# MasonFeurer/VoxelRayTracing

Hardware: AMD Instinct MI355X
Metric: Mrays/s at 1920x1080, 1 primary + 1 shadow ray (higher is better)
Workload: dtype f32

## Files before the change

### voxelraytracing_amd/csrc/vrt_kernels.hip

```cpp
#include <hip/hip_ext.h>

#include <atomic>

#include "vrt_tile.h"
#include "vrt_path_common.h"

namespace vrt {


template <int MARCH, bool LDS_ROOTS, bool STATS, bool SHADOW>
__global__ void __launch_bounds__(256) primary_tile_kernel(FrameParams P) {
    extern __shared__ uint32_t smem[];
    uint32_t *s_liquid = smem, *s_roots = smem + 24;
    unsigned long long *s_acc = reinterpret_cast<unsigned long long *>(smem + 8);
    uint32_t *s_hits = smem + 22;
    if (STATS && threadIdx.x < 6) s_acc[threadIdx.x] = 0ull;
    if (threadIdx.x == 0) *s_hits = 0u;
    stage_lds(P, s_roots, s_liquid, LDS_ROOTS);

    const uint32_t lane = threadIdx.x & 63u;
    uint32_t t_local = blockIdx.x * (blockDim.x >> 6) + (threadIdx.x >> 6);
    const bool live = t_local < P.tiles_local;
    if (!SHADOW && P.tile_order && live) t_local = P.tile_order[t_local];
    MarchResult R;
// ... 33 lines not shown
                    P.hits[blockIdx.x * 256u + base + rank] =
                        make_uint4(slot, __float_as_uint(so.x), __float_as_uint(so.y), __float_as_uint(so.z));
                }
            }
        }
        if (STATS && P.steps) P.steps[slot] = R.iters;
        if (!SHADOW && P.tile_cost) {
            uint32_t trips = R.trips;
#pragma unroll
            for (int o = 32; o > 0; o >>= 1) trips = max(trips, (uint32_t)__shfl_xor((int)trips, o, 64));
            if (lane == 0) P.tile_cost[t_local] = trips;
        }
    }
    if (STATS) {
        block_add(s_acc, 0, R.iters);
        block_add(s_acc, 1, R.visits);
        block_add(s_acc, 2, R.hit ? 1ull : 0ull);
    }
    if (SHADOW || STATS) {
        __syncthreads();
        if (threadIdx.x == 0) {
            if (SHADOW) P.blk_counts[blockIdx.x] = *s_hits;
            if (STATS) {
                atomicAdd(&P.counters[kCtrSteps], s_acc[0]);
                atomicAdd(&P.counters[kCtrVisits], s_acc[1]);
                atomicAdd(&P.counters[kCtrPrimarySteps], s_acc[0]);
                atomicAdd(&P.counters[kCtrPrimaryVisits], s_acc[1]);
                atomicAdd(&P.counters[kCtrHits], s_acc[2]);
            }
        }
    }
}

template <int MARCH, bool LDS_ROOTS, bool STATS>
__global__ void __launch_bounds__(256) shadow_kernel(FrameParams P) {
    extern __shared__ uint32_t smem[];
    uint32_t *s_liquid = smem, *s_roots = smem + 24;
    unsigned long long *s_acc = reinterpret_cast<unsigned long long *>(smem + 8);
    const uint32_t count = P.blk_counts[blockIdx.x];
    if (!STATS && count == 0u) return;
    if (STATS && threadIdx.x < 6) s_acc[threadIdx.x] = 0ull;
    stage_lds(P, s_roots, s_liquid, LDS_ROOTS);

    const bool active = threadIdx.x < count;
    if (!STATS && (threadIdx.x & ~63u) >= count) return;
    MarchResult R;
    R.iters = 0; R.visits = 0; R.hit = false;
    uint32_t slot = 0;
    if (active) {
        const uint4 rec = P.hits[blockIdx.x * 256u + threadIdx.x];
        slot = rec.x;
        const V3 so{__uint_as_float(rec.y), __uint_as_float(rec.z), __uint_as_float(rec.w)};
        const V3 sd = normalize_wave(V3{P.sun_local[0] - so.x, P.sun_local[1] - so.y, P.sun_local[2] - so.z});
        R = march<MARCH, LDS_ROOTS, STATS>(P, s_roots, s_liquid, so, sd);
        if (R.hit) {
            uint4 t = P.out[slot];
            t.x = __float_as_uint(__uint_as_float(t.x) * kShadowFactor);
            t.y = __float_as_uint(__uint_as_float(t.y) * kShadowFactor);
            t.z = __float_as_uint(__uint_as_float(t.z) * kShadowFactor);
            t.w |= VRT_ID_SHADOWED;
            P.out[slot] = t;
        }
        if (STATS && P.steps) P.steps[slot] |= R.iters << 16;
    }
    if (STATS) {
        block_add(s_acc, 0, active ? R.iters : 0u);
        block_add(s_acc, 1, active ? R.visits : 0u);
        __syncthreads();
        if (threadIdx.x == 0 && s_acc[0]) {
            atomicAdd(&P.counters[kCtrSteps], s_acc[0]);
            atomicAdd(&P.counters[kCtrVisits], s_acc[1]);
        }
    }
}


template <int MARCH, bool LDS_ROOTS, bool STATS, int WAVES, bool PROBE = false>
__global__ void __launch_bounds__(64 * WAVES) primary_shadow_wave_kernel(FrameParams P) {
    extern __shared__ uint32_t smem[];
    uint32_t *s_liquid = smem, *s_roots = smem + 24;
    unsigned long long *s_acc = reinterpret_cast<unsigned long long *>(smem + 8);
    if (STATS && threadIdx.x < 6) s_acc[threadIdx.x] = 0ull;
    unsigned long long t0 = 0, r0 = 0;
    if (PROBE) {
        t0 = __builtin_amdgcn_s_memtime();
        r0 = __builtin_amdgcn_s_memrealtime();
    }
    stage_lds(P, s_roots, s_liquid, LDS_ROOTS);

    const uint32_t lane = threadIdx.x & 63u;
    uint32_t t_local = blockIdx.x * (uint32_t)WAVES + (threadIdx.x >> 6);
    if (P.tile_order && t_local < P.tiles_local) t_local = P.tile_order[t_local];
    MarchResult R, S;
    R.iters = 0; R.visits = 0; R.hit = false;
    S.iters = 0; S.visits = 0; S.hit = false;
    R.trips = 0; S.trips = 0;
    if (t_local < P.tiles_local) {
        trace_tile<MARCH, LDS_ROOTS, STATS>(P, s_roots, s_liquid, t_local, lane, R, S);
        if (P.tile_cost) {
            uint32_t trips = R.trips + S.trips;
#pragma unroll
            for (int o = 32; o > 0; o >>= 1) trips = max(trips, (uint32_t)__shfl_xor((int)trips, o, 64));
            if (lane == 0) P.tile_cost[t_local] = trips;
        }
    }
    if (PROBE) {
        const unsigned long long t1 = __builtin_amdgcn_s_memtime(), r1 = __builtin_amdgcn_s_memrealtime();
// ... 546 lines not shown
```

### voxelraytracing_amd/csrc/vrt_march.h

```cpp
#pragma once

#include "vrt_device.h"


namespace vrt {

__device__ __forceinline__ int trunc2i(float x) {
    int r;
    asm("v_cvt_i32_f32 %0, %1" : "=v"(r) : "v"(x));
    return r;
}

constexpr uint32_t kBandLo = 0x30800000u;
constexpr uint32_t kBandSpan = 0x4E800000u - kBandLo;
__device__ __forceinline__ bool in_band(float x) { return (__float_as_uint(x) & 0x7FFFFFFFu) - kBandLo <= kBandSpan; }
__device__ __forceinline__ bool in_band3(V3 v) {
    const uint32_t a = (__float_as_uint(v.x) & 0x7FFFFFFFu) - kBandLo, b = (__float_as_uint(v.y) & 0x7FFFFFFFu) - kBandLo,
                   c = (__float_as_uint(v.z) & 0x7FFFFFFFu) - kBandLo;
    return max(max(a, b), c) <= kBandSpan;
}
__device__ __forceinline__ float rcp_refined(float d) {
    const float r = __builtin_amdgcn_rcpf(d);
    const float e = __builtin_fmaf(-d, r, 1.0f);
    return __builtin_fmaf(e, r, r);
// ... 341 lines not shown

__device__ __forceinline__ uint32_t mad_i24(int a, uint32_t uniform_b, uint32_t c) {
    uint32_t r;
    asm("v_mad_i32_i24 %0, %1, %2, %3" : "=v"(r) : "v"(a), "s"(uniform_b), "v"(c));
    return r;
}

__device__ __forceinline__ uint32_t bfi(uint32_t mask, uint32_t a, uint32_t b) {
    uint32_t r;
    asm("v_bitop3_b32 %0, %1, %2, %3 bitop3:0xca" : "=v"(r) : "v"(mask), "v"(a), "v"(b));
    return r;
}

template <uint32_t MASK>
__device__ __forceinline__ uint32_t low_bits_of(uint32_t a, uint32_t b) {
    static_assert(MASK <= 64u, "an inline constant");
    uint32_t r;
    asm("v_bitop3_b32 %0, %1, %2, %3 bitop3:0xca" : "=v"(r) : "n"(MASK), "v"(a), "v"(b));
    return r;
}
__device__ __forceinline__ uint32_t or_and(uint32_t a, uint32_t b, uint32_t c_mask_reg) {
    uint32_t r;
    asm("v_bitop3_b32 %0, %1, %2, %3 bitop3:0xf8" : "=v"(r) : "v"(a), "v"(b), "v"(c_mask_reg));
    return r;
}

__device__ __forceinline__ float abs_mul(float a, float b) {
    float r;
    asm("v_mul_f32_e64 %0, |%1|, %2" : "=v"(r) : "v"(a), "v"(b));
    return r;
}

__device__ __forceinline__ int flr2i(float x) {
    int r;
    asm("v_cvt_flr_i32_f32 %0, %1" : "=v"(r) : "v"(x));
    return r;
}
__device__ __forceinline__ float min3_f32(float a, float b, float c) {
    float r;
    asm("v_min3_f32 %0, %1, %2, %3" : "=v"(r) : "v"(a), "v"(b), "v"(c));
    return r;
}
__device__ __forceinline__ uint32_t min3_u32(uint32_t a, uint32_t b, uint32_t c) {
    uint32_t r;
    asm("v_min3_u32 %0, %1, %2, %3" : "=v"(r) : "v"(a), "v"(b), "v"(c));
    return r;
}

__device__ __forceinline__ bool finite3(V3 v) {
    return ((__float_as_uint(v.x) & 0x7F800000u) != 0x7F800000u) && ((__float_as_uint(v.y) & 0x7F800000u) != 0x7F800000u) &&
           ((__float_as_uint(v.z) & 0x7F800000u) != 0x7F800000u);
}

template <bool STATS, bool CAMERA = false>
__device__ __forceinline__ MarchResult march_grid(const FrameParams &P, const uint32_t *s_liquid, V3 origin, V3 dir) {
    MarchResult R;
    R.hit = false;
    R.pos = V3{0.f, 0.f, 0.f};
    R.norm = V3{0.f, 0.f, 0.f};
    R.water_dist = 0.0f;
    R.voxel = 0u;
    R.iters = 0u;
    R.visits = 0u;
    R.trips = 0u;

    const bool mx = dir.x >= 0.0f, my = dir.y >= 0.0f, mz = dir.z >= 0.0f;
    const bool careful = CAMERA ? ((P.cam_origin_facts & kCamNotFinite) != 0u || __ballot(!finite3(dir)) != 0ull)
                                : __ballot(!(finite3(origin) && finite3(dir))) != 0ull;

    V3 pos = origin;
    const bool nudge = CAMERA ? (P.cam_origin_facts & kCamOnPlane) != 0u
                              : (pos.x - floorf(pos.x) < 0.001f || pos.y - floorf(pos.y) < 0.001f || pos.z - floorf(pos.z) < 0.001f);
    if (nudge) {
        pos.x += 0.001f * dir.x;
        pos.y += 0.001f * dir.y;
        pos.z += 0.001f * dir.z;
    }
    const float world_max = P.world_max;
    if (CAMERA && !(P.cam_origin_facts & kCamOnPlane)) {
        if (P.cam_origin_facts & kCamOutside) return R;
    } else if ((pos.x <= 0.0f || pos.y <= 0.0f || pos.z <= 0.0f) || (pos.x >= world_max || pos.y >= world_max || pos.z >= world_max))
        return R;

    const V3 unit = unit_steps(dir);
    float ux = fabsf(unit.x), uy = fabsf(unit.y), uz = fabsf(unit.z);
    asm("" : "+v"(ux), "+v"(uy), "+v"(uz));
    constexpr uint32_t kTwo23 = 0x4B000000u;
    uint32_t mxm = kTwo23 | (mx ? 0x007FFFFFu : 0u), mym = kTwo23 | (my ? 0x007FFFFFu : 0u), mzm = kTwo23 | (mz ? 0x007FFFFFu : 0u);
    float cx = mx ? -8388607.0f : -8388608.0f, cy = my ? -8388607.0f : -8388608.0f, cz = mz ? -8388607.0f : -8388608.0f;
    asm("" : "+v"(mxm), "+v"(mym), "+v"(mzm));

    const uint32_t wsize = P.world.size;
    const TableBuf gb = table_buffer(P.grid, P.grid_bytes), bb = table_buffer(P.bricks, P.brick_bytes);
    const TableBuf bb16 = __builtin_amdgcn_make_buffer_rsrc(const_cast<uint16_t *>(P.bricks), 2, P.brick_bytes / 2u, 0x00020000);
    uint32_t liq_lo = P.liquid_lo, liq_span = P.liquid_span;
    if (!P.liquid_is_range) { liq_lo = 1u; liq_span = 0xFFFFFFFEu; }
    else if (liq_lo == 0u) { if (liq_span) { liq_lo = 1u; liq_span -= 1u; } else liq_lo = 0x80000000u; }
    const uint32_t row_bytes = (P.grid_dim + 1u) * 4u, slab_bytes = (P.grid_dim + 1u) * row_bytes;

    int vx = trunc2i(pos.x), vy = trunc2i(pos.y), vz = trunc2i(pos.z);
    uint32_t voxel = 0u;
    float step = -1.0f, adx = 0.0f, ady = 0.0f, adz = 0.0f;
    float dew = -1.0f;
    constexpr uint32_t kPlain = kAirLeaf, kSlow = 0xFFFFFFFFu;
    uint32_t slow_below = careful ? kSlow : kPlain;
    float total_len = 0.0f;
    uint32_t iter = 0u;
    uint32_t looked_up = 0u;

    auto take_step = [&](uint32_t sel) __attribute__((always_inline)) {
        const float tx = (__uint_as_float(bfi(sel, mxm, (uint32_t)vx)) + cx) - pos.x;
        const float ty = (__uint_as_float(bfi(sel, mym, (uint32_t)vy)) + cy) - pos.y;
        const float tz = (__uint_as_float(bfi(sel, mzm, (uint32_t)vz)) + cz) - pos.z;
        adx = abs_mul(tx, ux);
        ady = abs_mul(ty, uy);
        adz = abs_mul(tz, uz);
        step = min3_f32(adx, ady, adz);
        if (__ballot(!(step > 0.0f)) != 0ull)
            step = __uint_as_float(min3_u32(__float_as_uint(adx) - 1u, __float_as_uint(ady) - 1u, __float_as_uint(adz) - 1u) + 1u);
        total_len += step;
        const float sp = step + 0.001f;
        pos.x += dir.x * (step == adx ? sp : step);
        pos.y += dir.y * (step == ady ? sp : step);
        pos.z += dir.z * (step == adz ? sp : step);
        vx = flr2i(pos.x);
        vy = flr2i(pos.y);
        vz = flr2i(pos.z);
    };
    auto lookup = [&]() __attribute__((always_inline)) {
        return (uint32_t)__builtin_amdgcn_raw_buffer_load_b32(
            gb, mad_i24(vz >> 2, slab_bytes, mad_i24(vy >> 2, row_bytes, (uint32_t)vx & ~3u)), 0, 0);
    };

    for (;;) {
        uint32_t e;
        if constexpr (!STATS) {
            uint32_t t0, t1, t2;
            unsigned long long sa, sb, sx, sd, sn, sw, fy, fz;
            uint32_t parked;
            uint32_t trips = __builtin_amdgcn_readfirstlane(iter) - kMaxSteps;
            asm volatile(
                "s_mov_b64 %[sd], 0\n\t"
                "s_setprio 1\n\t"
                "v_cmp_ne_u32_e64 %[sw], %[kair], %[below]\n"
                ".Lvrt_step_%=:\n\t"
                "v_ashrrev_i32_e32 %[t1], 2, %[vy]\n\t"
                "v_and_b32_e32 %[t2], -4, %[vx]\n\t"
                "v_mad_i32_i24 %[t1], %[t1], %[row], %[t2]\n\t"
                "v_ashrrev_i32_e32 %[t0], 2, %[vz]\n\t"
                "v_mad_i32_i24 %[t0], %[t0], %[slab], %[t1]\n\t"
                "buffer_load_dword %[e], %[t0], %[desc], 0 offen\n\t"
                "s_waitcnt vmcnt(0)\n\t"
                "v_cmp_lt_u32_e32 vcc, %[e], %[below]\n\t"
                "s_cbranch_vccnz .Lvrt_split_%=\n"
                ".Lvrt_planes_%=:\n\t"
                "v_bitop3_b32 %[ax], %[e], %[mx], %[vx] bitop3:0xca\n\t"
                "v_bitop3_b32 %[ay], %[e], %[my], %[vy] bitop3:0xca\n\t"
                "v_bitop3_b32 %[az], %[e], %[mz], %[vz] bitop3:0xca\n\t"
                "v_add_f32_e32 %[ax], %[cx], %[ax]\n\t"
                "v_add_f32_e32 %[ay], %[cy], %[ay]\n\t"
                "v_add_f32_e32 %[az], %[cz], %[az]\n\t"
                "v_sub_f32_e32 %[ax], %[ax], %[px]\n\t"
                "v_sub_f32_e32 %[ay], %[ay], %[py]\n\t"
                "v_sub_f32_e32 %[az], %[az], %[pz]\n\t"
                "v_mul_f32_e64 %[ax], |%[ax]|, %[ux]\n\t"
                "v_mul_f32_e64 %[ay], |%[ay]|, %[uy]\n\t"
                "v_mul_f32_e64 %[az], |%[az]|, %[uz]\n\t"
                "v_min3_f32 %[st], %[ax], %[ay], %[az]\n\t"
                "v_cmp_nlt_f32_e32 vcc, 0, %[st]\n\t"
                "s_cbranch_vccnz .Lvrt_zero_%=\n"
                ".Lvrt_move_%=:\n\t"
                "v_cmp_eq_f32_e32 vcc, %[st], %[ax]\n\t"
                "v_add_f32_e32 %[t0], 0x3a83126f, %[st]\n\t"
                "v_cmp_eq_f32_e64 %[fy], %[st], %[ay]\n\t"
                "v_add_f32_e32 %[tl], %[tl], %[st]\n\t"
                "v_cndmask_b32_e32 %[t1], %[st], %[t0], vcc\n\t"
                "v_mul_f32_e32 %[t1], %[dx], %[t1]\n\t"
                "v_cmp_eq_f32_e64 %[fz], %[st], %[az]\n\t"
                "v_add_f32_e32 %[px], %[px], %[t1]\n\t"
                "v_cndmask_b32_e64 %[t2], %[st], %[t0], %[fy]\n\t"
                "v_mul_f32_e32 %[t2], %[dy], %[t2]\n\t"
                "v_cndmask_b32_e64 %[t0], %[st], %[t0], %[fz]\n\t"
                "v_add_f32_e32 %[py], %[py], %[t2]\n\t"
                "v_cvt_flr_i32_f32_e32 %[vx], %[px]\n\t"
                "v_mul_f32_e32 %[t0], %[dz], %[t0]\n\t"
                "v_cvt_flr_i32_f32_e32 %[vy], %[py]\n\t"
                "v_add_f32_e32 %[pz], %[pz], %[t0]\n\t"
                "v_cvt_flr_i32_f32_e32 %[vz], %[pz]\n\t"
                "s_add_u32 %[it], %[it], 1\n\t"
                "s_cbranch_scc0 .Lvrt_step_%=\n\t"
                "s_branch .Lvrt_out_%=\n"
                ".Lvrt_zero_%=:\n\t"
                "v_add_u32_e32 %[t0], -1, %[ax]\n\t"
                "v_add_u32_e32 %[t1], -1, %[ay]\n\t"
                "v_add_u32_e32 %[t2], -1, %[az]\n\t"
                "v_min3_u32 %[t0], %[t0], %[t1], %[t2]\n\t"
                "v_add_u32_e32 %[st], 1, %[t0]\n\t"
                "s_branch .Lvrt_move_%=\n"
                ".Lvrt_split_%=:\n\t"
                "s_cmp_lg_u64 %[sw], 0\n\t"
                "s_cbranch_scc1 .Lvrt_out_%=\n\t"
                "s_and_saveexec_b64 %[sx], vcc\n\t"
                "v_cmp_gt_i32_e32 vcc, 0, %[e]\n\t"
                "s_and_saveexec_b64 %[sa], vcc\n\t"
                "s_andn2_b64 %[sn], %[sa], exec\n\t"
                "s_cbranch_execz .Lvrt_decide_%=\n\t"
                "v_lshlrev_b32_e32 %[t0], 2, %[vy]\n\t"
                "v_lshlrev_b32_e32 %[t1], 4, %[vz]\n\t"
                "v_bitop3_b32 %[t0], 3, %[vx], %[t0] bitop3:0xca\n\t"
                "v_bitop3_b32 %[t0], 15, %[t0], %[t1] bitop3:0xca\n\t"
                "v_bitop3_b32 %[t0], %[kbrick], %[e], %[t0] bitop3:0xca\n\t"
                "buffer_load_ushort %[t1], %[t0], %[bdesc], 0 idxen\n\t"
                "s_waitcnt vmcnt(0)\n\t"
                "v_cmp_lt_u32_e32 vcc, 1, %[t1]\n\t"
                "s_or_b64 %[sb], %[sn], vcc\n\t"
                "s_cbranch_scc1 .Lvrt_decide_%=\n\t"
                "v_and_or_b32 %[e], %[t1], 1, %[kair]\n\t"
                "s_mov_b64 exec, %[sx]\n\t"
                "s_branch .Lvrt_planes_%=\n"
                ".Lvrt_decide_%=:\n\t"
                "v_lshrrev_b32_e32 %[t2], 1, %[t1]\n\t"
                "s_mov_b64 exec, %[sn]\n\t"
                "v_lshrrev_b32_e32 %[t2], 16, %[e]\n\t"
                "s_mov_b64 exec, %[sa]\n\t"
                "v_subrev_u32_e32 %[t0], %[liqlo], %[t2]\n\t"
                "v_cmp_ge_u32_e32 vcc, %[liqspan], %[t0]\n\t"
                "s_cbranch_vccnz .Lvrt_leave_%=\n\t"
                "v_cmp_ne_u32_e32 vcc, 0, %[t2]\n\t"
                "v_cmp_eq_u32_e64 %[sb], 0, %[e]\n\t"
                "s_or_b64 %[sb], %[sb], vcc\n\t"
                "s_or_b64 %[sd], %[sd], %[sb]\n\t"
                "s_andn2_b64 exec, %[sa], %[sb]\n\t"
                "v_and_or_b32 %[e], %[t1], 1, %[kair]\n\t"
                "s_mov_b64 exec, %[sb]\n\t"
                "v_mov_b32_e32 %[vox], %[t2]\n\t"
                "s_andn2_b64 exec, %[sx], %[sb]\n\t"
                "s_cbranch_scc1 .Lvrt_planes_%=\n\t"
                "s_branch .Lvrt_out_%=\n"
                ".Lvrt_leave_%=:\n\t"
                "s_mov_b64 exec, %[sx]\n"
                ".Lvrt_out_%=:\n\t"
                "s_setprio 0\n\t"
                "s_or_b64 exec, exec, %[sd]\n\t"
                "v_cndmask_b32_e64 %[parked], 0, 1, %[sd]"
                : [px] "+v"(pos.x), [py] "+v"(pos.y), [pz] "+v"(pos.z), [tl] "+v"(total_len), [vx] "+v"(vx), [vy] "+v"(vy), [vz] "+v"(vz),
                  [st] "+v"(step), [ax] "+v"(adx), [ay] "+v"(ady), [az] "+v"(adz), [e] "=&v"(e), [it] "+s"(trips),
                  [t0] "=&v"(t0), [t1] "=&v"(t1), [t2] "=&v"(t2), [sa] "=&s"(sa), [sb] "=&s"(sb), [sx] "=&s"(sx), [sd] "=&s"(sd), [sn] "=&s"(sn), [sw] "=&s"(sw),
                  [fy] "=&s"(fy), [fz] "=&s"(fz),
                  [vox] "+v"(voxel), [parked] "=&v"(parked)
                : [mx] "v"(mxm), [my] "v"(mym), [mz] "v"(mzm), [cx] "v"(cx), [cy] "v"(cy), [cz] "v"(cz), [ux] "v"(ux), [uy] "v"(uy), [uz] "v"(uz),
                  [dx] "v"(dir.x), [dy] "v"(dir.y), [dz] "v"(dir.z), [below] "v"(slow_below), [desc] "s"(gb), [row] "s"(row_bytes), [slab] "s"(slab_bytes),
                  [bdesc] "s"(bb16), [kair] "s"(kAirLeaf), [kbrick] "s"(0x7FFFFFC0u), [liqlo] "s"(liq_lo), [liqspan] "s"(liq_span)
                : "vcc", "scc", "memory");
            iter = trips + kMaxSteps;
            if (parked) break;
            if (iter >= kMaxSteps) break;
        } else {
            bool exhausted = false;
            for (;;) {
                e = lookup();
                if (__ballot(e < slow_below) != 0ull) break;
                iter += 1u;
                if (STATS) { looked_up += 1u; R.visits += (uint32_t)__clz((int)((e & 31u) + 1u)) - 25u; }
                take_step(e);
                if (iter >= kMaxSteps) { exhausted = true; break; }
            }
            if (exhausted) break;
        }
        iter += 1u;
        uint32_t lo = e;
        bool stop = false;
        if (e < slow_below) {
            if (careful) {
                vx = trunc2i(pos.x);
                vy = trunc2i(pos.y);
                vz = trunc2i(pos.z);
                e = 0u;
                if (!(min3_nan_ignoring(pos.x, pos.y, pos.z) < 0.0f || max(max((uint32_t)vx, (uint32_t)vy), (uint32_t)vz) >= wsize))
                    e = lookup();
                lo = e;
            }
            stop = e == 0u;
            if (!stop) {
                voxel = 0u;
                if (is_split_entry(e)) {
                    const uint32_t u = ((uint32_t)vx & 3u) | (((uint32_t)vy & 3u) << 2) | (((uint32_t)vz & 3u) << 4);
                    const uint32_t b = (uint32_t)__builtin_amdgcn_raw_buffer_load_b16(bb, (e + u) << 1, 0, 0);
                    lo = kAirLeaf | (b & 1u);
                    voxel = b >> 1;
                } else if (e < kAirLeaf) {
                    lo = kAirLeaf | (e & 31u);
                    voxel = e >> 16;
                }
                if (STATS) { looked_up += 1u; R.visits += (uint32_t)__clz((int)((lo & 31u) + 1u)) - 25u; }
                if (voxel != 0u) {
                    if (!is_liquid_ranged(P, s_liquid, voxel)) stop = true;
                    else if (dew == -1.0f) { dew = total_len; slow_below = kSlow; }
                } else if (dew != -1.0f) {
                    R.water_dist += total_len - dew;
                    dew = -1.0f;
                    if (!careful) slow_below = kPlain;
                }
            }
        } else if (STATS) {
            looked_up += 1u;
            R.visits += (uint32_t)__clz((int)((lo & 31u) + 1u)) - 25u;
        }
        if (stop) break;
        take_step(lo);
        if (iter >= kMaxSteps) break;
    }
    R.iters = STATS ? looked_up : 0u;
    R.trips = iter;
    if (dew != -1.0f) R.water_dist += total_len - dew;
    if (min3_nan_ignoring(pos.x, pos.y, pos.z) < 0.0f ||
        max(max((uint32_t)trunc2i(pos.x), (uint32_t)trunc2i(pos.y)), (uint32_t)trunc2i(pos.z)) >= wsize)
        return R;
    const bool stepped = step != -1.0f;

    R.hit = true;
    R.pos = pos;
    if (stepped)
        R.norm = V3{(step == adx ? 1.0f : 0.0f) * -vsign(dir.x), (step == ady ? 1.0f : 0.0f) * -vsign(dir.y),
                    (step == adz ? 1.0f : 0.0f) * -vsign(dir.z)};
    R.voxel = voxel;
    return R;
}

template <int MARCH, bool LDS_ROOTS, bool STATS = false, bool CAMERA = false>
__device__ __forceinline__ MarchResult march(const FrameParams &P, const uint32_t *s_roots, const uint32_t *s_liquid,
                                             V3 origin, V3 dir) {
    if (MARCH == 1) return march_literal<LDS_ROOTS>(P, s_roots, s_liquid, origin, dir);
    if (MARCH == 2) return march_fast<LDS_ROOTS>(P, s_roots, s_liquid, origin, dir);
    return march_grid<STATS, CAMERA>(P, s_liquid, origin, dir);
}

template <bool CAM_ORIGIN = false, bool NO_DISC = false>
__device__ __forceinline__ V3 ray_sky(const FrameParams &P, V3 origin, V3 dir) {
    const float ground_to_sky_t = vsmoothstep(-0.01f, 0.0f, dir.y);
    const float sky_gradient_t = __builtin_amdgcn_exp2f(0.35f * __builtin_amdgcn_logf(vsmoothstep(0.0f, 0.4f, dir.y)));
    const V3 grad{vmix(1.0f, P.settings.sky_color[0], sky_gradient_t), vmix(0.3f, P.settings.sky_color[1], sky_gradient_t),
                  vmix(0.0f, P.settings.sky_color[2], sky_gradient_t)};
    const V3 sun_dir = CAM_ORIGIN ? V3{P.cam_sun_dir[0], P.cam_sun_dir[1], P.cam_sun_dir[2]}
                                  : normalize_wave(V3{P.sun_local[0] - origin.x, P.sun_local[1] - origin.y, P.sun_local[2] - origin.z});
    const float sun = (vdot(dir, sun_dir) > (1.0f - 0.01f) && ground_to_sky_t >= 1.0f) ? 1.0f : 0.0f;
    const float add = sun * (NO_DISC ? 0.0f : P.settings.sun_intensity);
    return V3{vmix(0.03f, grad.x, ground_to_sky_t) + add, vmix(0.03f, grad.y, ground_to_sky_t) + add,
              vmix(0.03f, grad.z, ground_to_sky_t) + add};
}

__device__ __forceinline__ void create_ray(const FrameParams &P, int sx, int sy, V3 &origin, V3 &dir) {
    const float x = P.ndc_x[sx];
    const float y = P.ndc_y[sy];
    const float c0 = x, c1 = -y, c2 = -1.0f, c3 = 1.0f;
    const float *ip = P.cam.inv_proj_mat;
    const float e0 = c0 * ip[0] + c1 * ip[1] + c2 * ip[2] + c3 * ip[3];
    const float e1 = c0 * ip[4] + c1 * ip[5] + c2 * ip[6] + c3 * ip[7];
    const float *iv = P.cam.inv_view_mat;
    const float e2 = -1.0f, e3 = 0.0f;
    const V3 w{e0 * iv[0] + e1 * iv[1] + e2 * iv[2] + e3 * iv[3], e0 * iv[4] + e1 * iv[5] + e2 * iv[6] + e3 * iv[7],
               e0 * iv[8] + e1 * iv[9] + e2 * iv[10] + e3 * iv[11]};
    dir = normalize_wave(w);
    origin = V3{P.cam_origin[0], P.cam_origin[1], P.cam_origin[2]};
}

template <bool EXACT_SKY>
__device__ __forceinline__ uint32_t shade(const FrameParams &P, const MarchResult &R, V3 origin, V3 dir, V3 &color) {
    V3 mc{0.f, 0.f, 0.f};
    if (R.hit) {
        const vrt_material *m = &P.mats[min(R.voxel, 255u)];
        mc = V3{m->color[0], m->color[1], m->color[2]};
        if (R.norm.x != 0.0f) { mc.x *= 0.5f; mc.y *= 0.5f; mc.z *= 0.5f; }
        if (R.norm.z != 0.0f) { mc.x *= 0.7f; mc.y *= 0.7f; mc.z *= 0.7f; }
        if (R.norm.y == -1.0f) { mc.x *= 0.2f; mc.y *= 0.2f; mc.z *= 0.2f; }
        if (P.settings.show_step_count == 1u) {
            const float f = vclamp((float)R.iters / 500.0f, 0.0f, 1.0f);
            mc = V3{f, f, f};
        }
    }
    if (EXACT_SKY || !P.finite_settings) {
        const V3 sky = ray_sky<true>(P, origin, dir);
        const float fh = R.hit ? 1.0f : 0.0f, fm = R.hit ? 0.0f : 1.0f;
        color = V3{mc.x * fh + sky.x * fm, mc.y * fh + sky.y * fm, mc.z * fh + sky.z * fm};
    } else if (R.hit) {
        color = mc;
    } else {
        color = ray_sky<true>(P, origin, dir);
// ... 38 lines not shown
```

### voxelraytracing_amd/csrc/vrt_tile.h

```cpp
#pragma once

#include "vrt_march.h"

namespace vrt {

__device__ __forceinline__ uint32_t unorm8(float x) { return (uint32_t)rintf(vclamp(x, 0.0f, 1.0f) * 255.0f) & 0xFFu; }

struct PresentSample { int x0, x1, y0, y1; float a, b, mask; };
__device__ __forceinline__ PresentSample present_sample(uint32_t w, uint32_t h, uint32_t screen_w, uint32_t screen_h, const vrt_crosshair &ch, uint32_t sx, uint32_t sy,
                                                        bool in_box) {
    const float ssx = (float)screen_w, ssy = (float)screen_h;
    const float cx = ssx * 0.5f, cy = ssy * 0.5f;
    const float u = ((float)sx + 0.5f) / ssx, v = ((float)sy + 0.5f) / ssy;
    const float px = u * ssx, py = v * ssy;
    PresentSample S;
    S.mask = 0.0f;
    if (in_box && ch.style == 1u) {
        const float dx = cx - px, dy = cy - py;
        S.mask = (sqrtf(dx * dx + dy * dy) < ch.size ? 1.0f : 0.0f) * ch.color[3];
    }
    if (in_box && ch.style == 2u) {
        const float dx = fabsf(cx - px), dy = fabsf(cy - py);
        const float wd = ch.size * 0.25f;
        S.mask = (((dx < ch.size && dy < wd) || (dy < ch.size && dx < wd)) ? 1.0f : 0.0f) * ch.color[3];
// ... 31 lines not shown
#pragma unroll
    for (int k = 0; k < 4; k++) q |= unorm8(texel[k] * (1.0f - S.mask) + cc[k] * S.mask) << (8 * k);
    return q;
}

__device__ __forceinline__ void store_screen(const FrameParams &P, uint32_t px, uint32_t py, V3 color) {
    const uint32_t qr = unorm8(color.x), qg = unorm8(color.y), qb = unorm8(color.z);
    uint32_t q = 0xFF000000u | qr | (qg << 8) | (qb << 16);
    const uint32_t tx0 = __builtin_amdgcn_readfirstlane(px & ~7u), ty0 = __builtin_amdgcn_readfirstlane(py & ~7u);
    if (P.present_box[0] < P.present_box[1] && tx0 < P.present_box[1] && tx0 + 8u > P.present_box[0] && ty0 < P.present_box[3] && ty0 + 8u > P.present_box[2]) {
        const bool in_box = px >= P.present_box[0] && px < P.present_box[1] && py >= P.present_box[2] && py < P.present_box[3];
        const PresentSample S = present_sample(P.width, P.height, P.width, P.height, P.crosshair, px, py, in_box);
        const float own[3] = {(float)qr / 255.0f, (float)qg / 255.0f, (float)qb / 255.0f};
        const int l00 = ((S.y0 & 7) << 3) | (S.x0 & 7), l10 = ((S.y0 & 7) << 3) | (S.x1 & 7), l01 = ((S.y1 & 7) << 3) | (S.x0 & 7), l11 = ((S.y1 & 7) << 3) | (S.x1 & 7);
        float v00[4], v10[4], v01[4], v11[4];
#pragma unroll
        for (int k = 0; k < 3; k++) {
            v00[k] = __shfl(own[k], l00, 64); v10[k] = __shfl(own[k], l10, 64);
            v01[k] = __shfl(own[k], l01, 64); v11[k] = __shfl(own[k], l11, 64);
        }
        v00[3] = v10[3] = v01[3] = v11[3] = 1.0f;
        if (in_box) q = present_blend(S, P.crosshair, v00, v10, v01, v11);
    }
    __builtin_nontemporal_store(q, &P.screen[py * P.width + px]);
}

__device__ __forceinline__ void store_pixel(const FrameParams &P, uint32_t slot, uint32_t px, uint32_t py, V3 color, uint32_t id, const MarchResult &R) {
    if (P.compact)
        reinterpret_cast<uint2 *>(P.out)[slot] = make_uint2(id | (R.norm.y < 0.0f ? kIdNormYNeg : 0u), __float_as_uint(R.water_dist));
    else if (!P.screen_only)
        store_streaming(&P.out[slot], make_uint4(__float_as_uint(color.x), __float_as_uint(color.y), __float_as_uint(color.z), id));
    if (P.screen) store_screen(P, px, py, color);
}

template <int MARCH, bool LDS_ROOTS, bool STATS>
__device__ __forceinline__ void trace_tile(const FrameParams &P, const uint32_t *s_roots, const uint32_t *s_liquid, uint32_t t_local,
                                           uint32_t lane, MarchResult &R, MarchResult &S) {
    const uint32_t tile = shard_tile(t_local, P.shard_first, P.shard_run, P.shard_period);
    uint32_t px, py;
    tile_pixel(P, tile, lane, px, py);
    const uint32_t slot = P.tile_major ? t_local * 64u + lane : py * P.width + px;

    V3 origin, dir;
    create_ray(P, (int)px, (int)py, origin, dir);
    R = march<MARCH, LDS_ROOTS, STATS, true>(P, s_roots, s_liquid, origin, dir);
    V3 color;
    uint32_t id = shade<MARCH == 1>(P, R, origin, dir, color);

    const bool launch = R.hit && R.voxel != 0u && !is_liquid(s_liquid, R.voxel);
    if (launch) {
        id |= VRT_ID_SHADOW_RAY;
        const V3 so{R.pos.x + R.norm.x * kShadowBias, R.pos.y + R.norm.y * kShadowBias, R.pos.z + R.norm.z * kShadowBias};
        const V3 sd = normalize_wave(V3{P.sun_local[0] - so.x, P.sun_local[1] - so.y, P.sun_local[2] - so.z});
        S = march<MARCH, LDS_ROOTS, STATS>(P, s_roots, s_liquid, so, sd);
        if (S.hit) {
            color.x *= kShadowFactor;
            color.y *= kShadowFactor;
            color.z *= kShadowFactor;
            id |= VRT_ID_SHADOWED;
        }
    }
    store_pixel(P, slot, px, py, color, id, R);
    if (STATS && P.steps) P.steps[slot] = R.iters | (S.iters << 16);
    const unsigned long long ballot = __ballot(launch);
    if (lane == 0) P.blk_counts[t_local] = (uint32_t)__popcll(ballot);
}

}
```

Before: 57510.

## Add hit-only march variant for shadow rays skipping water and normal bookkeeping

Adds a HIT_ONLY template path to the grid marcher, used by both shadow ray call sites, that only reports whether an opaque voxel was hit. The inline-asm loop is turned into a macro with two instantiations: the hit-only one drops total-length accumulation, water-distance tracking and the wet-region transition code, and exits early without computing position and normal. This trims per-step ALU work and register pressure in the shadow march, at the cost of a second, more complex hand-written asm variant whose exec-mask logic must stay correct.

```diff
diff --git a/voxelraytracing_amd/csrc/vrt_kernels.hip b/voxelraytracing_amd/csrc/vrt_kernels.hip
--- a/voxelraytracing_amd/csrc/vrt_kernels.hip
+++ b/voxelraytracing_amd/csrc/vrt_kernels.hip
@@ -109,7 +109,7 @@
         slot = rec.x;
         const V3 so{__uint_as_float(rec.y), __uint_as_float(rec.z), __uint_as_float(rec.w)};
         const V3 sd = normalize_wave(V3{P.sun_local[0] - so.x, P.sun_local[1] - so.y, P.sun_local[2] - so.z});
-        R = march<MARCH, LDS_ROOTS, STATS>(P, s_roots, s_liquid, so, sd);
+        R = march<MARCH, LDS_ROOTS, STATS, false, true>(P, s_roots, s_liquid, so, sd);
         if (R.hit) {
             uint4 t = P.out[slot];
             t.x = __float_as_uint(__uint_as_float(t.x) * kShadowFactor);
diff --git a/voxelraytracing_amd/csrc/vrt_march.h b/voxelraytracing_amd/csrc/vrt_march.h
--- a/voxelraytracing_amd/csrc/vrt_march.h
+++ b/voxelraytracing_amd/csrc/vrt_march.h
@@ -417,8 +417,210 @@
            ((__float_as_uint(v.z) & 0x7F800000u) != 0x7F800000u);
 }
 
-template <bool STATS, bool CAMERA = false>
+#define VRT_STEP_LEN_FULL "v_add_f32_e32 %[tl], %[tl], %[st]\n\t"
+#define VRT_STEP_LEN_HIT ""
+#define VRT_STEP_SW_FULL "s_cbranch_scc1 .Lvrt_wet_%=\n\t"
+#define VRT_STEP_SW_HIT "s_cbranch_scc1 .Lvrt_out_%=\n\t"
+#define VRT_STEP_DECIDE_FULL                                                                                                          \
+    "s_cbranch_vccnz .Lvrt_leave_%=\n\t"                                                                                              \
+    "v_cmp_ne_u32_e32 vcc, 0, %[t2]\n\t"                                                                                   \
+    "v_cmp_eq_u32_e64 %[sb], 0, %[e]\n\t"                                                                             \
+    "s_or_b64 %[sb], %[sb], vcc\n\t"                                                                    \
+    "s_or_b64 %[sd], %[sd], %[sb]\n\t"                                                                                                \
+    "s_andn2_b64 exec, %[sa], %[sb]\n\t"                                                                \
+    "v_and_or_b32 %[e], %[t1], 1, %[kair]\n\t"                                                  \
+    "s_mov_b64 exec, %[sb]\n\t"                                                                                                       \
+    "v_mov_b32_e32 %[vox], %[t2]\n\t"
+#define VRT_STEP_DECIDE_HIT                                                                                                           \
+    "s_mov_b64 %[fy], vcc\n\t"                                                                                       \
+    "s_and_b64 vcc, vcc, %[gm]\n\t"                                                                                                   \
+    "s_cbranch_vccnz .Lvrt_leave_%=\n\t"                                                                                              \
+    "v_cmp_ne_u32_e32 vcc, 0, %[t2]\n\t"                                                                             \
+    "v_cmp_eq_u32_e64 %[sb], 0, %[e]\n\t"                                                                             \
+    "s_andn2_b64 vcc, vcc, %[fy]\n\t"                                                                \
+    "s_or_b64 %[sb], %[sb], vcc\n\t"                                                                    \
+    "s_or_b64 %[sd], %[sd], %[sb]\n\t"                                                                                                \
+    "s_andn2_b64 exec, %[sn], %[sb]\n\t"                                                                     \
+    "v_and_or_b32 %[e], %[e], 31, %[kair]\n\t"                                                               \
+    "s_or_b64 %[fz], %[sn], %[sb]\n\t"                                                                                                \
+    "s_andn2_b64 exec, %[sa], %[fz]\n\t"                                                 \
+    "v_and_or_b32 %[e], %[t1], 1, %[kair]\n\t"
+#define VRT_STEP_WET_FULL                                                                                                             \
+    ".Lvrt_wet_%=:\n\t"                                                                                                               \
+    "s_cmp_lg_u64 %[gm], 0\n\t"                                  \
+    "s_cbranch_scc1 .Lvrt_out_%=\n\t"                                                                                                 \
+    "s_mov_b64 %[sx], exec\n\t"                                                                                                       \
+    "s_mov_b64 %[sb], 0\n\t"                                                                                                          \
+    "v_mov_b32_e32 %[t2], 0\n\t"                                                 \
+    "v_cmp_gt_u32_e32 vcc, %[kair], %[e]\n\t"                                                                                         \
+    "s_and_saveexec_b64 %[sn], vcc\n\t"                                                             \
+    "s_cbranch_execz .Lvrt_book_%=\n\t"                                                                                               \
+    "v_cmp_gt_i32_e32 vcc, 0, %[e]\n\t"                                                                                               \
+    "s_and_saveexec_b64 %[sa], vcc\n\t"                                                       \
+    "s_cbranch_execz .Lvrt_wleaf_%=\n\t"                                                                                              \
+    "v_lshlrev_b32_e32 %[t0], 2, %[vy]\n\t"                                              \
+    "v_lshlrev_b32_e32 %[t1], 4, %[vz]\n\t"                                                                                           \
+    "v_bitop3_b32 %[t0], 3, %[vx], %[t0] bitop3:0xca\n\t"                                                                             \
+    "v_bitop3_b32 %[t0], 15, %[t0], %[t1] bitop3:0xca\n\t"                                                                            \
+    "v_bitop3_b32 %[t0], %[kbrick], %[e], %[t0] bitop3:0xca\n\t"                                                                      \
+    "buffer_load_ushort %[t1], %[t0], %[bdesc], 0 idxen\n\t"                                                                          \
+    "s_waitcnt vmcnt(0)\n\t"                                                                                                          \
+    "v_lshrrev_b32_e32 %[t2], 1, %[t1]\n\t"                                                         \
+    "v_and_or_b32 %[e], %[t1], 1, %[kair]\n"                                         \
+    ".Lvrt_wleaf_%=:\n\t"                                                                                                             \
+    "s_andn2_b64 exec, %[sa], exec\n\t"                                                       \
+    "v_cmp_eq_u32_e64 %[sb], 0, %[e]\n\t"                                                                   \
+    "v_lshrrev_b32_e32 %[t2], 16, %[e]\n\t"                                                                  \
+    "v_and_or_b32 %[e], %[e], 31, %[kair]\n"                                                                        \
+    ".Lvrt_book_%=:\n\t"                                                                                                              \
+    "s_mov_b64 exec, %[sx]\n\t"                                                                                                       \
+    "v_subrev_u32_e32 %[t0], %[liqlo], %[t2]\n\t"                                                                                     \
+    "v_cmp_ge_u32_e64 %[fy], %[liqspan], %[t0]\n\t"                                        \
+    "v_cmp_ne_u32_e32 vcc, 0, %[t2]\n\t"                                                                                              \
+    "v_mov_b32_e32 %[vox], %[t2]\n\t"                                                \
+    "s_andn2_b64 vcc, vcc, %[fy]\n\t"                                                                                      \
+    "s_or_b64 %[sb], %[sb], vcc\n\t"                                                                    \
+    "s_or_b64 %[sd], %[sd], %[sb]\n\t"                                                                                                \
+    "s_and_b64 %[sw], %[sw], %[sx]\n\t"                                           \
+    "s_andn2_b64 exec, %[fy], %[sw]\n\t"                                               \
+    "v_mov_b32_e32 %[dew], %[tl]\n\t"                                                                                                 \
+    "v_mov_b32_e32 %[below], -1\n\t"                                                                                                  \
+    "s_or_b64 %[fz], %[fy], %[sb]\n\t"                                                                                                \
+    "s_andn2_b64 exec, %[sw], %[fz]\n\t"                                                        \
+    "v_sub_f32_e32 %[t0], %[tl], %[dew]\n\t"                                                                                          \
+    "v_add_f32_e32 %[wd], %[wd], %[t0]\n\t"                                                                                           \
+    "v_mov_b32_e32 %[dew], -1.0\n\t"                                                                                                  \
+    "v_mov_b32_e32 %[below], %[kair]\n\t"                                                                                             \
+    "s_andn2_b64 exec, %[sx], %[sb]\n\t"                                                                 \
+    "s_cbranch_scc0 .Lvrt_out_%=\n\t"                                                                 \
+    "v_cmp_ne_u32_e64 %[sw], %[kair], %[below]\n\t"                                                       \
+    "s_branch .Lvrt_planes_%=\n"
+#define VRT_STEP_WET_HIT ""
+#define VRT_STEP_OUTS_FULL , [tl] "+v"(total_len), [vox] "+v"(voxel), [dew] "+v"(dew), [wd] "+v"(R.water_dist), [below] "+v"(slow_below)
+#define VRT_STEP_INS_FULL
+#define VRT_STEP_OUTS_HIT
+#define VRT_STEP_INS_HIT , [below] "v"(slow_below)
+
+#define VRT_MARCH_LOOP(LEN, SW, DECIDE, WET, OUTS, INS)                                                                               \
+    asm volatile(                                                                                                                     \
+        "s_mov_b64 %[sd], 0\n\t"                                                                                                      \
+        "s_setprio 1\n\t"                                            \
+        "v_cmp_ne_u32_e64 %[sw], %[kair], %[below]\n"                                             \
+        ".Lvrt_step_%=:\n\t"                                                                                                          \
+        "v_ashrrev_i32_e32 %[t1], 2, %[vy]\n\t"                                                                                       \
+        "v_and_b32_e32 %[t2], -4, %[vx]\n\t"                                                                                          \
+        "v_mad_i32_i24 %[t1], %[t1], %[row], %[t2]\n\t"                                                                               \
+        "v_ashrrev_i32_e32 %[t0], 2, %[vz]\n\t"                                                                                       \
+        "v_mad_i32_i24 %[t0], %[t0], %[slab], %[t1]\n\t"                                                                              \
+        "buffer_load_dword %[e], %[t0], %[desc], 0 offen\n\t"                                                                         \
+        "s_waitcnt vmcnt(0)\n\t"                                                                                                      \
+        "v_cmp_lt_u32_e32 vcc, %[e], %[below]\n\t"                                                                                    \
+        "s_cbranch_vccnz .Lvrt_split_%=\n"                                                  \
+        ".Lvrt_planes_%=:\n\t"                                                                                                        \
+        "v_bitop3_b32 %[ax], %[e], %[mx], %[vx] bitop3:0xca\n\t"                \
+        "v_bitop3_b32 %[ay], %[e], %[my], %[vy] bitop3:0xca\n\t"                                                                      \
+        "v_bitop3_b32 %[az], %[e], %[mz], %[vz] bitop3:0xca\n\t"                                                                      \
+        "v_add_f32_e32 %[ax], %[cx], %[ax]\n\t"                                                                                       \
+        "v_add_f32_e32 %[ay], %[cy], %[ay]\n\t"                                                                                       \
+        "v_add_f32_e32 %[az], %[cz], %[az]\n\t"                                                                                       \
+        "v_sub_f32_e32 %[ax], %[ax], %[px]\n\t"                                                                                       \
+        "v_sub_f32_e32 %[ay], %[ay], %[py]\n\t"                                                                                       \
+        "v_sub_f32_e32 %[az], %[az], %[pz]\n\t"                                                                                       \
+        "v_mul_f32_e64 %[ax], |%[ax]|, %[ux]\n\t"                                                                          \
+        "v_mul_f32_e64 %[ay], |%[ay]|, %[uy]\n\t"                                                                                     \
+        "v_mul_f32_e64 %[az], |%[az]|, %[uz]\n\t"                                                                                     \
+        "v_min3_f32 %[st], %[ax], %[ay], %[az]\n\t"                                                                          \
+        "v_cmp_nlt_f32_e32 vcc, 0, %[st]\n\t"                                                                                         \
+        "s_cbranch_vccnz .Lvrt_zero_%=\n"                                     \
+        ".Lvrt_move_%=:\n\t"                                                                                                          \
+         \
+         \
+                \
+                               \
+        "v_cmp_eq_f32_e32 vcc, %[st], %[ax]\n\t"                                                                                      \
+        "v_add_f32_e32 %[t0], 0x3a83126f, %[st]\n\t"                                                                \
+        "v_cmp_eq_f32_e64 %[fy], %[st], %[ay]\n\t"                                                                                    \
+        LEN                                                                                                                           \
+        "v_cndmask_b32_e32 %[t1], %[st], %[t0], vcc\n\t"                                                                              \
+        "v_mul_f32_e32 %[t1], %[dx], %[t1]\n\t"                                                                                       \
+        "v_cmp_eq_f32_e64 %[fz], %[st], %[az]\n\t"                                                                                    \
+        "v_add_f32_e32 %[px], %[px], %[t1]\n\t"                                                                                       \
+        "v_cndmask_b32_e64 %[t2], %[st], %[t0], %[fy]\n\t"                                                                            \
+        "v_mul_f32_e32 %[t2], %[dy], %[t2]\n\t"                                                                                       \
+        "v_cndmask_b32_e64 %[t0], %[st], %[t0], %[fz]\n\t"                                                                            \
+        "v_add_f32_e32 %[py], %[py], %[t2]\n\t"                                                                                       \
+        "v_cvt_flr_i32_f32_e32 %[vx], %[px]\n\t"                                                                                      \
+        "v_mul_f32_e32 %[t0], %[dz], %[t0]\n\t"                                                                                       \
+        "v_cvt_flr_i32_f32_e32 %[vy], %[py]\n\t"                                                                                      \
+        "v_add_f32_e32 %[pz], %[pz], %[t0]\n\t"                                                                                       \
+        "v_cvt_flr_i32_f32_e32 %[vz], %[pz]\n\t"                                                                                      \
+        "s_add_u32 %[it], %[it], 1\n\t"                                         \
+        "s_cbranch_scc0 .Lvrt_step_%=\n\t"                                                                                            \
+        "s_branch .Lvrt_out_%=\n"                                                                                                     \
+        ".Lvrt_zero_%=:\n\t"                                                                                                          \
+        "v_add_u32_e32 %[t0], -1, %[ax]\n\t"                                                                                          \
+        "v_add_u32_e32 %[t1], -1, %[ay]\n\t"                                                                                          \
+        "v_add_u32_e32 %[t2], -1, %[az]\n\t"                                                                                          \
+        "v_min3_u32 %[t0], %[t0], %[t1], %[t2]\n\t"                                                                                   \
+        "v_add_u32_e32 %[st], 1, %[t0]\n\t"                                                                                           \
+        "s_branch .Lvrt_move_%=\n"                                                                                                    \
+         \
+             \
+             \
+                \
+                  \
+             \
+        ".Lvrt_split_%=:\n\t"                                                                                                         \
+        "s_cmp_lg_u64 %[sw], 0\n\t"                                                            \
+        SW                                                                                                                            \
+        "s_and_saveexec_b64 %[sx], vcc\n\t"                          \
+        "v_cmp_gt_i32_e32 vcc, 0, %[e]\n\t"                                                                                           \
+        "s_and_saveexec_b64 %[sa], vcc\n\t"                                                             \
+        "s_andn2_b64 %[sn], %[sa], exec\n\t"                                \
+        "s_cbranch_execz .Lvrt_decide_%=\n\t"                                                                                         \
+        "v_lshlrev_b32_e32 %[t0], 2, %[vy]\n\t"                                              \
+        "v_lshlrev_b32_e32 %[t1], 4, %[vz]\n\t"                                                                                       \
+        "v_bitop3_b32 %[t0], 3, %[vx], %[t0] bitop3:0xca\n\t"                                                                         \
+        "v_bitop3_b32 %[t0], 15, %[t0], %[t1] bitop3:0xca\n\t"                                           \
+        "v_bitop3_b32 %[t0], %[kbrick], %[e], %[t0] bitop3:0xca\n\t"   \
+        "buffer_load_ushort %[t1], %[t0], %[bdesc], 0 idxen\n\t"                                                                      \
+        "s_waitcnt vmcnt(0)\n\t"                                                                                                      \
+        "v_cmp_lt_u32_e32 vcc, 1, %[t1]\n\t"                                            \
+        "s_or_b64 %[sb], %[sn], vcc\n\t"                                                                                              \
+        "s_cbranch_scc1 .Lvrt_decide_%=\n\t"                                                    \
+        "v_and_or_b32 %[e], %[t1], 1, %[kair]\n\t"                   \
+        "s_mov_b64 exec, %[sx]\n\t"                                                                                                   \
+        "s_branch .Lvrt_planes_%=\n"                                                                                                  \
+        ".Lvrt_decide_%=:\n\t"                                                                                                        \
+        "v_lshrrev_b32_e32 %[t2], 1, %[t1]\n\t"                                                 \
+        "s_mov_b64 exec, %[sn]\n\t"                                                                                                   \
+        "v_lshrrev_b32_e32 %[t2], 16, %[e]\n\t"                                                    \
+        "s_mov_b64 exec, %[sa]\n\t"                                                                                                   \
+        "v_subrev_u32_e32 %[t0], %[liqlo], %[t2]\n\t"                                                                                 \
+        "v_cmp_ge_u32_e32 vcc, %[liqspan], %[t0]\n\t"                                         \
+        DECIDE                                                                                                                        \
+        "s_andn2_b64 exec, %[sx], %[sb]\n\t"                                                             \
+        "s_cbranch_scc1 .Lvrt_planes_%=\n\t"                                                                                          \
+        "s_branch .Lvrt_out_%=\n"                                                                     \
+        ".Lvrt_leave_%=:\n\t"                                                                                                         \
+        "s_mov_b64 exec, %[sx]\n"                                                                                                     \
+        WET                                                                                                                           \
+        ".Lvrt_out_%=:\n\t"                                                                                                           \
+        "s_setprio 0\n\t"                                                                                                             \
+        "s_or_b64 exec, exec, %[sd]\n\t"                                                                                              \
+        "v_cndmask_b32_e64 %[parked], 0, 1, %[sd]"                                                                                    \
+        : [px] "+v"(pos.x), [py] "+v"(pos.y), [pz] "+v"(pos.z), [vx] "+v"(vx), [vy] "+v"(vy), [vz] "+v"(vz),                          \
+          [st] "+v"(step), [ax] "+v"(adx), [ay] "+v"(ady), [az] "+v"(adz), [e] "=&v"(e), [it] "+s"(trips),                            \
+          [t0] "=&v"(t0), [t1] "=&v"(t1), [t2] "=&v"(t2), [sa] "=&s"(sa), [sb] "=&s"(sb), [sx] "=&s"(sx), [sd] "=&s"(sd), [sn] "=&s"(sn), [sw] "=&s"(sw), \
+          [fy] "=&s"(fy), [fz] "=&s"(fz), [parked] "=&v"(parked) OUTS                                                                 \
+        : [mx] "v"(mxm), [my] "v"(mym), [mz] "v"(mzm), [cx] "v"(cx), [cy] "v"(cy), [cz] "v"(cz), [ux] "v"(ux), [uy] "v"(uy), [uz] "v"(uz), \
+          [dx] "v"(dir.x), [dy] "v"(dir.y), [dz] "v"(dir.z), [desc] "s"(gb), [row] "s"(row_bytes), [slab] "s"(slab_bytes),            \
+          [bdesc] "s"(bb16), [kair] "s"(kAirLeaf), [kbrick] "s"(0x7FFFFFC0u), [liqlo] "s"(liq_lo), [liqspan] "s"(liq_span), [gm] "s"(gm) INS \
+        : "vcc", "scc", "memory")
+
+template <bool STATS, bool CAMERA = false, bool HIT_ONLY = false>
 __device__ __forceinline__ MarchResult march_grid(const FrameParams &P, const uint32_t *s_liquid, V3 origin, V3 dir) {
+    constexpr bool HIT = HIT_ONLY && !STATS;
     MarchResult R;
     R.hit = false;
     R.pos = V3{0.f, 0.f, 0.f};
@@ -504,119 +706,12 @@
             unsigned long long sa, sb, sx, sd, sn, sw, fy, fz;
             uint32_t parked;
             uint32_t trips = __builtin_amdgcn_readfirstlane(iter) - kMaxSteps;
-            asm volatile(
-                "s_mov_b64 %[sd], 0\n\t"
-                "s_setprio 1\n\t"
-                "v_cmp_ne_u32_e64 %[sw], %[kair], %[below]\n"
-                ".Lvrt_step_%=:\n\t"
-                "v_ashrrev_i32_e32 %[t1], 2, %[vy]\n\t"
-                "v_and_b32_e32 %[t2], -4, %[vx]\n\t"
-                "v_mad_i32_i24 %[t1], %[t1], %[row], %[t2]\n\t"
-                "v_ashrrev_i32_e32 %[t0], 2, %[vz]\n\t"
-                "v_mad_i32_i24 %[t0], %[t0], %[slab], %[t1]\n\t"
-                "buffer_load_dword %[e], %[t0], %[desc], 0 offen\n\t"
-                "s_waitcnt vmcnt(0)\n\t"
-                "v_cmp_lt_u32_e32 vcc, %[e], %[below]\n\t"
-                "s_cbranch_vccnz .Lvrt_split_%=\n"
-                ".Lvrt_planes_%=:\n\t"
-                "v_bitop3_b32 %[ax], %[e], %[mx], %[vx] bitop3:0xca\n\t"
-                "v_bitop3_b32 %[ay], %[e], %[my], %[vy] bitop3:0xca\n\t"
-                "v_bitop3_b32 %[az], %[e], %[mz], %[vz] bitop3:0xca\n\t"
-                "v_add_f32_e32 %[ax], %[cx], %[ax]\n\t"
-                "v_add_f32_e32 %[ay], %[cy], %[ay]\n\t"
-                "v_add_f32_e32 %[az], %[cz], %[az]\n\t"
-                "v_sub_f32_e32 %[ax], %[ax], %[px]\n\t"
-                "v_sub_f32_e32 %[ay], %[ay], %[py]\n\t"
-                "v_sub_f32_e32 %[az], %[az], %[pz]\n\t"
-                "v_mul_f32_e64 %[ax], |%[ax]|, %[ux]\n\t"
-                "v_mul_f32_e64 %[ay], |%[ay]|, %[uy]\n\t"
-                "v_mul_f32_e64 %[az], |%[az]|, %[uz]\n\t"
-                "v_min3_f32 %[st], %[ax], %[ay], %[az]\n\t"
-                "v_cmp_nlt_f32_e32 vcc, 0, %[st]\n\t"
-                "s_cbranch_vccnz .Lvrt_zero_%=\n"
-                ".Lvrt_move_%=:\n\t"
-                "v_cmp_eq_f32_e32 vcc, %[st], %[ax]\n\t"
-                "v_add_f32_e32 %[t0], 0x3a83126f, %[st]\n\t"
-                "v_cmp_eq_f32_e64 %[fy], %[st], %[ay]\n\t"
-                "v_add_f32_e32 %[tl], %[tl], %[st]\n\t"
-                "v_cndmask_b32_e32 %[t1], %[st], %[t0], vcc\n\t"
-                "v_mul_f32_e32 %[t1], %[dx], %[t1]\n\t"
-                "v_cmp_eq_f32_e64 %[fz], %[st], %[az]\n\t"
-                "v_add_f32_e32 %[px], %[px], %[t1]\n\t"
-                "v_cndmask_b32_e64 %[t2], %[st], %[t0], %[fy]\n\t"
-                "v_mul_f32_e32 %[t2], %[dy], %[t2]\n\t"
-                "v_cndmask_b32_e64 %[t0], %[st], %[t0], %[fz]\n\t"
-                "v_add_f32_e32 %[py], %[py], %[t2]\n\t"
-                "v_cvt_flr_i32_f32_e32 %[vx], %[px]\n\t"
-                "v_mul_f32_e32 %[t0], %[dz], %[t0]\n\t"
-                "v_cvt_flr_i32_f32_e32 %[vy], %[py]\n\t"
-                "v_add_f32_e32 %[pz], %[pz], %[t0]\n\t"
-                "v_cvt_flr_i32_f32_e32 %[vz], %[pz]\n\t"
-                "s_add_u32 %[it], %[it], 1\n\t"
-                "s_cbranch_scc0 .Lvrt_step_%=\n\t"
-                "s_branch .Lvrt_out_%=\n"
-                ".Lvrt_zero_%=:\n\t"
-                "v_add_u32_e32 %[t0], -1, %[ax]\n\t"
-                "v_add_u32_e32 %[t1], -1, %[ay]\n\t"
-                "v_add_u32_e32 %[t2], -1, %[az]\n\t"
-                "v_min3_u32 %[t0], %[t0], %[t1], %[t2]\n\t"
-                "v_add_u32_e32 %[st], 1, %[t0]\n\t"
-                "s_branch .Lvrt_move_%=\n"
-                ".Lvrt_split_%=:\n\t"
-                "s_cmp_lg_u64 %[sw], 0\n\t"
-                "s_cbranch_scc1 .Lvrt_out_%=\n\t"
-                "s_and_saveexec_b64 %[sx], vcc\n\t"
-                "v_cmp_gt_i32_e32 vcc, 0, %[e]\n\t"
-                "s_and_saveexec_b64 %[sa], vcc\n\t"
-                "s_andn2_b64 %[sn], %[sa], exec\n\t"
-                "s_cbranch_execz .Lvrt_decide_%=\n\t"
-                "v_lshlrev_b32_e32 %[t0], 2, %[vy]\n\t"
-                "v_lshlrev_b32_e32 %[t1], 4, %[vz]\n\t"
-                "v_bitop3_b32 %[t0], 3, %[vx], %[t0] bitop3:0xca\n\t"
-                "v_bitop3_b32 %[t0], 15, %[t0], %[t1] bitop3:0xca\n\t"
-                "v_bitop3_b32 %[t0], %[kbrick], %[e], %[t0] bitop3:0xca\n\t"
-                "buffer_load_ushort %[t1], %[t0], %[bdesc], 0 idxen\n\t"
-                "s_waitcnt vmcnt(0)\n\t"
-                "v_cmp_lt_u32_e32 vcc, 1, %[t1]\n\t"
-                "s_or_b64 %[sb], %[sn], vcc\n\t"
-                "s_cbranch_scc1 .Lvrt_decide_%=\n\t"
-                "v_and_or_b32 %[e], %[t1], 1, %[kair]\n\t"
-                "s_mov_b64 exec, %[sx]\n\t"
-                "s_branch .Lvrt_planes_%=\n"
-                ".Lvrt_decide_%=:\n\t"
-                "v_lshrrev_b32_e32 %[t2], 1, %[t1]\n\t"
-                "s_mov_b64 exec, %[sn]\n\t"
-                "v_lshrrev_b32_e32 %[t2], 16, %[e]\n\t"
-                "s_mov_b64 exec, %[sa]\n\t"
-                "v_subrev_u32_e32 %[t0], %[liqlo], %[t2]\n\t"
-                "v_cmp_ge_u32_e32 vcc, %[liqspan], %[t0]\n\t"
-                "s_cbranch_vccnz .Lvrt_leave_%=\n\t"
-                "v_cmp_ne_u32_e32 vcc, 0, %[t2]\n\t"
-                "v_cmp_eq_u32_e64 %[sb], 0, %[e]\n\t"
-                "s_or_b64 %[sb], %[sb], vcc\n\t"
-                "s_or_b64 %[sd], %[sd], %[sb]\n\t"
-                "s_andn2_b64 exec, %[sa], %[sb]\n\t"
-                "v_and_or_b32 %[e], %[t1], 1, %[kair]\n\t"
-                "s_mov_b64 exec, %[sb]\n\t"
-                "v_mov_b32_e32 %[vox], %[t2]\n\t"
-                "s_andn2_b64 exec, %[sx], %[sb]\n\t"
-                "s_cbranch_scc1 .Lvrt_planes_%=\n\t"
-                "s_branch .Lvrt_out_%=\n"
-                ".Lvrt_leave_%=:\n\t"
-                "s_mov_b64 exec, %[sx]\n"
-                ".Lvrt_out_%=:\n\t"
-                "s_setprio 0\n\t"
-                "s_or_b64 exec, exec, %[sd]\n\t"
-                "v_cndmask_b32_e64 %[parked], 0, 1, %[sd]"
-                : [px] "+v"(pos.x), [py] "+v"(pos.y), [pz] "+v"(pos.z), [tl] "+v"(total_len), [vx] "+v"(vx), [vy] "+v"(vy), [vz] "+v"(vz),
-                  [st] "+v"(step), [ax] "+v"(adx), [ay] "+v"(ady), [az] "+v"(adz), [e] "=&v"(e), [it] "+s"(trips),
-                  [t0] "=&v"(t0), [t1] "=&v"(t1), [t2] "=&v"(t2), [sa] "=&s"(sa), [sb] "=&s"(sb), [sx] "=&s"(sx), [sd] "=&s"(sd), [sn] "=&s"(sn), [sw] "=&s"(sw),
-                  [fy] "=&s"(fy), [fz] "=&s"(fz),
-                  [vox] "+v"(voxel), [parked] "=&v"(parked)
-                : [mx] "v"(mxm), [my] "v"(mym), [mz] "v"(mzm), [cx] "v"(cx), [cy] "v"(cy), [cz] "v"(cz), [ux] "v"(ux), [uy] "v"(uy), [uz] "v"(uz),
-                  [dx] "v"(dir.x), [dy] "v"(dir.y), [dz] "v"(dir.z), [below] "v"(slow_below), [desc] "s"(gb), [row] "s"(row_bytes), [slab] "s"(slab_bytes),
-                  [bdesc] "s"(bb16), [kair] "s"(kAirLeaf), [kbrick] "s"(0x7FFFFFC0u), [liqlo] "s"(liq_lo), [liqspan] "s"(liq_span)
-                : "vcc", "scc", "memory");
+            const uint32_t gmw = __builtin_amdgcn_readfirstlane(((!HIT && careful) || !P.liquid_is_range) ? ~0u : 0u);
+            const unsigned long long gm = ((unsigned long long)gmw << 32) | gmw;
+            if constexpr (HIT)
+                VRT_MARCH_LOOP(VRT_STEP_LEN_HIT, VRT_STEP_SW_HIT, VRT_STEP_DECIDE_HIT, VRT_STEP_WET_HIT, VRT_STEP_OUTS_HIT, VRT_STEP_INS_HIT);
+            else
+                VRT_MARCH_LOOP(VRT_STEP_LEN_FULL, VRT_STEP_SW_FULL, VRT_STEP_DECIDE_FULL, VRT_STEP_WET_FULL, VRT_STEP_OUTS_FULL, VRT_STEP_INS_FULL);
             iter = trips + kMaxSteps;
             if (parked) break;
             if (iter >= kMaxSteps) break;
@@ -660,8 +755,8 @@
                 if (STATS) { looked_up += 1u; R.visits += (uint32_t)__clz((int)((lo & 31u) + 1u)) - 25u; }
                 if (voxel != 0u) {
                     if (!is_liquid_ranged(P, s_liquid, voxel)) stop = true;
-                    else if (dew == -1.0f) { dew = total_len; slow_below = kSlow; }
-                } else if (dew != -1.0f) {
+                    else if (!HIT && dew == -1.0f) { dew = total_len; slow_below = kSlow; }
+                } else if (!HIT && dew != -1.0f) {
                     R.water_dist += total_len - dew;
                     dew = -1.0f;
                     if (!careful) slow_below = kPlain;
@@ -677,13 +772,14 @@
     }
     R.iters = STATS ? looked_up : 0u;
     R.trips = iter;
-    if (dew != -1.0f) R.water_dist += total_len - dew;
+    if (!HIT && dew != -1.0f) R.water_dist += total_len - dew;
     if (min3_nan_ignoring(pos.x, pos.y, pos.z) < 0.0f ||
         max(max((uint32_t)trunc2i(pos.x), (uint32_t)trunc2i(pos.y)), (uint32_t)trunc2i(pos.z)) >= wsize)
         return R;
+    R.hit = true;
+    if (HIT) return R;
     const bool stepped = step != -1.0f;
 
-    R.hit = true;
     R.pos = pos;
     if (stepped)
         R.norm = V3{(step == adx ? 1.0f : 0.0f) * -vsign(dir.x), (step == ady ? 1.0f : 0.0f) * -vsign(dir.y),
@@ -692,12 +788,12 @@
     return R;
 }
 
-template <int MARCH, bool LDS_ROOTS, bool STATS = false, bool CAMERA = false>
+template <int MARCH, bool LDS_ROOTS, bool STATS = false, bool CAMERA = false, bool HIT_ONLY = false>
 __device__ __forceinline__ MarchResult march(const FrameParams &P, const uint32_t *s_roots, const uint32_t *s_liquid,
                                              V3 origin, V3 dir) {
     if (MARCH == 1) return march_literal<LDS_ROOTS>(P, s_roots, s_liquid, origin, dir);
     if (MARCH == 2) return march_fast<LDS_ROOTS>(P, s_roots, s_liquid, origin, dir);
-    return march_grid<STATS, CAMERA>(P, s_liquid, origin, dir);
+    return march_grid<STATS, CAMERA, HIT_ONLY>(P, s_liquid, origin, dir);
 }
 
 template <bool CAM_ORIGIN = false, bool NO_DISC = false>
diff --git a/voxelraytracing_amd/csrc/vrt_tile.h b/voxelraytracing_amd/csrc/vrt_tile.h
--- a/voxelraytracing_amd/csrc/vrt_tile.h
+++ b/voxelraytracing_amd/csrc/vrt_tile.h
@@ -107,7 +107,7 @@
         id |= VRT_ID_SHADOW_RAY;
         const V3 so{R.pos.x + R.norm.x * kShadowBias, R.pos.y + R.norm.y * kShadowBias, R.pos.z + R.norm.z * kShadowBias};
         const V3 sd = normalize_wave(V3{P.sun_local[0] - so.x, P.sun_local[1] - so.y, P.sun_local[2] - so.z});
-        S = march<MARCH, LDS_ROOTS, STATS>(P, s_roots, s_liquid, so, sd);
+        S = march<MARCH, LDS_ROOTS, STATS, false, true>(P, s_roots, s_liquid, so, sd);
         if (S.hit) {
             color.x *= kShadowFactor;
             color.y *= kShadowFactor;
```

Result: no change. 57410 (-0.2%).
